# PRBonn/kinematic-icp

Hardware: AMD Instinct MI355X
Metric: scans/sec (ICP registration only), 128k-pt scan vs 1M-pt map (higher is better)
Workload: dtype f64; 1 GPU; cfg2: 131072-pt 64-beam scan vs 986360-pt / 74758-voxel map, voxel 1.00 m, tau 0.6708 m, default ICP iterations (mean 1.00 per scan); one step = one kicp_register_device_batch call = 3200 independent scans against the fixed map, up to 8 in flight at a time (every scan's result bit-identical to registering it alone); 64 distinct scans cycled; scans_in_flight=8, distinct_scans=64, points_per_gpu=131072, parallelism=single GPU

## Files before the change

kinematic_icp_amd/csrc/kicp_kernels.hpp:

```cpp
#pragma once
#include <cfloat>
#include <climits>

#include "kicp_common.hpp"
#include "kicp_se3.hpp"

namespace kicp {

constexpr int kMaxLog = 32;
constexpr int kNumSums = 7;
constexpr int kNumLimbs = 3 * kNumSums;
constexpr int kReduceWords = 24;
constexpr double kFixScale = 1099511627776.0;
constexpr double kFixLimit = 8796093022208.0;

struct HostRecord {
    unsigned long long seq;
    int32_t done, iter, converged, nan_flag;
    Pose T;
    double beta;
    double log_ncorr[kMaxLog];
    double log_sums[kMaxLog][6];
    double log_dx[kMaxLog][2];
    double sums[kNumSums];
// ... 66 lines not shown
    return sp;
}

struct PassParams {
    const double *src;
    uint32_t n;
    MapView map;
    double tau;
    SearchParams search;
    IcpState *st;
    unsigned long long *partials;
    unsigned int *tickets;
    unsigned long long *group_acc;
    SolveParams sol;
    int32_t dbg;
    int32_t *corr_index;
    double *corr_d2, *corr_nn;
};
#ifdef KICP_DBG_BUILD
constexpr bool kDbgBuild = true;
#else
constexpr bool kDbgBuild = false;
#endif
__device__ __forceinline__ bool dbg_is(const PassParams &p, int v) { return kDbgBuild && p.dbg == v; }
__device__ __forceinline__ bool dbg_not(const PassParams &p, int v) { return !kDbgBuild || p.dbg != v; }


struct I128 {
    unsigned long long lo;
    long long hi;
// ... 363 lines not shown
}

__device__ __forceinline__ int wave_sum_to_lane63(int v) {
    v += __builtin_amdgcn_update_dpp(0, v, 0x111, 0xF, 0xF, true);
    v += __builtin_amdgcn_update_dpp(0, v, 0x112, 0xF, 0xF, true);
    v += __builtin_amdgcn_update_dpp(0, v, 0x114, 0xF, 0xF, true);
    v += __builtin_amdgcn_update_dpp(0, v, 0x118, 0xF, 0xF, true);
    v += __builtin_amdgcn_update_dpp(0, v, 0x142, 0xA, 0xF, true);
    v += __builtin_amdgcn_update_dpp(0, v, 0x143, 0xC, 0xF, true);
    return v;
}

constexpr unsigned long long kGaveUpUnit = 1ull << 16;
constexpr unsigned long long kLostRowUnit = 1ull << 8;
constexpr long long kRowWaitTicks = 200000000ll;
__device__ __forceinline__ void counting_hand_over(const I128 &t, int range_error, int gave_up, const PassParams &p, uint32_t row_tag, uint32_t acc_set,
                                                   uint32_t row_set, int lane, uint32_t nblocks = gridDim.x) {
    const uint32_t b = blockIdx.x, g = b / kGroup, ngroups = (nblocks + kGroup - 1) / kGroup;
    long long l[3] = {0ll, 0ll, 0ll};
    if (lane < kNumSums) i128_to_limbs(t, l);
    const int from = min(lane, kNumLimbs - 1) / 3;
    const long long a0 = __shfl(l[0], from, 64), a1 = __shfl(l[1], from, 64), a2 = __shfl(l[2], from, 64);
    long long word = lane % 3 == 0 ? a0 : (lane % 3 == 1 ? a1 : a2);
    if (lane >= kNumLimbs) word = lane == kNumLimbs ? static_cast<long long>(range_error) + (gave_up ? static_cast<long long>(kGaveUpUnit) : 0ll) : 0ll;
    if (lane < kReduceWords) {
        const uint32_t group_size = min(static_cast<uint32_t>(kGroup), nblocks - g * kGroup);
        unsigned long long *acc = p.group_acc + (static_cast<size_t>(acc_set) * ngroups + g) * kAccStride + lane;
        const unsigned long long mine = static_cast<unsigned long long>(word + kAccBias);
        const unsigned long long old = __hip_atomic_fetch_add(acc, (1ull << kAccCountShift) + mine, __ATOMIC_RELAXED, __HIP_MEMORY_SCOPE_AGENT);
        if ((old >> kAccCountShift) == group_size - 1u) {
            const long long total = static_cast<long long>((old & ((1ull << kAccCountShift) - 1ull)) + mine) - static_cast<long long>(group_size) * kAccBias;
            __hip_atomic_store(acc, 0ull, __ATOMIC_RELAXED, __HIP_MEMORY_SCOPE_AGENT);
            __hip_atomic_store(p.sol.pub_rows + (static_cast<size_t>(row_set) * ngroups + g) * kReduceWords + lane,
                               (static_cast<unsigned long long>(total) << 16) | static_cast<unsigned long long>(row_tag), __ATOMIC_RELAXED, __HIP_MEMORY_SCOPE_SYSTEM);
        }
    }
}

template <int BLOCK, bool ROWS_ONLY = false>
__device__ __forceinline__ void finish_pass(Acc &a, const PassParams &p, int (*s_red)[kWaveLimbs], int *s_flag, uint32_t row_tag, int gave_up = 0,
                                            uint32_t parity = 0u, uint32_t nblocks = gridDim.x) {
    const int lane = threadIdx.x & 63, wave = threadIdx.x >> 6;
    IcpState *st = p.st;
    if (!ROWS_ONLY && dbg_is(p, 8)) {
        if (p.sol.mode == 4 && wave == 0 && blockIdx.x % kGroup == 0 && lane < kReduceWords)
            __hip_atomic_store(p.sol.pub_rows + static_cast<size_t>(blockIdx.x / kGroup) * kReduceWords + lane, static_cast<unsigned long long>(p.sol.tag),
                               __ATOMIC_RELAXED, __HIP_MEMORY_SCOPE_SYSTEM);
        if (blockIdx.x == 0 && wave == 0 && p.sol.mode == 2) {
            if (lane < kReduceWords) __hip_atomic_store(p.sol.pub_words + lane, 0ll, __ATOMIC_RELAXED, __HIP_MEMORY_SCOPE_SYSTEM);
            asm volatile("s_waitcnt vmcnt(0)" ::: "memory");
            if (lane == 0) __hip_atomic_store(p.sol.pub_seq, p.sol.pub_value, __ATOMIC_RELAXED, __HIP_MEMORY_SCOPE_SYSTEM);
        }
        return;
    }
    int range_error = a.range_error;
    int limb[kWaveLimbs];
    if (dbg_is(p, 10) || dbg_is(p, 12)) {
#pragma unroll
        for (int k = 0; k < kWaveLimbs; ++k) limb[k] = wave_sum_to_lane63(a.limb[k]);
    } else {
        const unsigned long long holders = __ballot(a.limb[6 * kTermLimbs + 1] != 0);
        const int n_holders = __popcll(holders);
        const int some = holders ? static_cast<int>(__ffsll(static_cast<long long>(holders))) - 1 : 0;
#pragma unroll
        for (int k = 0; k < kTermLimbs; ++k) limb[k] = n_holders * __builtin_amdgcn_readlane(a.limb[k], some);
        limb[6 * kTermLimbs] = 0, limb[6 * kTermLimbs + 1] = n_holders << 19, limb[6 * kTermLimbs + 2] = 0, limb[6 * kTermLimbs + 3] = 0;
        int w10[10], x5[5];
        const bool p0 = (lane & 1) != 0, p1 = (lane & 2) != 0;
#pragma unroll
        for (int j = 0; j < 10; ++j) {
            const int lo = a.limb[kTermLimbs + 2 * j], hi = a.limb[kTermLimbs + 2 * j + 1];
            w10[j] = (p0 ? hi : lo) + __builtin_amdgcn_update_dpp(0, p0 ? lo : hi, 0xB1, 0xF, 0xF, true);
        }
#pragma unroll
        for (int j = 0; j < 5; ++j) {
            const int lo = w10[2 * j], hi = w10[2 * j + 1];
            x5[j] = (p1 ? hi : lo) + __builtin_amdgcn_update_dpp(0, p1 ? lo : hi, 0x4E, 0xF, 0xF, true);
        }
#pragma unroll
        for (int j = 0; j < 5; ++j) x5[j] += __builtin_amdgcn_update_dpp(0, x5[j], 0x114, 0xF, 0xF, true);
// ... 13 lines not shown
            for (int k = 0; k < kTermLimbs; ++k) s_red[wave][k] = limb[k], s_red[wave][6 * kTermLimbs + k] = limb[6 * kTermLimbs + k];
            if (range_error) atomicOr(s_flag, 2);
        }
    }
    if (dbg_is(p, 10) || dbg_is(p, 12)) {
        range_error = __any(range_error) ? 1 : 0;
        if (lane == 63) {
#pragma unroll
            for (int k = 0; k < kWaveLimbs; ++k) s_red[wave][k] = limb[k];
            if (range_error) atomicOr(s_flag, 2);
        }
    }
    __syncthreads();
    if (wave != 0) return;
    range_error = (*s_flag & 2) ? 1 : 0;
    I128 t{0ull, 0ll};
    if (lane < kNumSums) {
        for (int w = 0; w < BLOCK / 64; ++w)
            i128_add_limb_sums(t, s_red[w][kTermLimbs * lane], s_red[w][kTermLimbs * lane + 1], s_red[w][kTermLimbs * lane + 2], s_red[w][kTermLimbs * lane + 3]);
    }
    const uint32_t b = blockIdx.x, g = b / kGroup, ngroups = (nblocks + kGroup - 1) / kGroup;
    const bool counting = ROWS_ONLY || (p.sol.mode == 4 && dbg_not(p, 14));
    if (!ROWS_ONLY && counting) parity = row_tag & 1u;
    if (counting) {
        counting_hand_over(t, range_error, gave_up, p, row_tag, parity, ROWS_ONLY ? parity : 0u, lane, nblocks);
        return;
    }
    unsigned long long *const rows0 = p.partials + (ROWS_ONLY ? static_cast<size_t>(parity) * nblocks * kReduceWords : 0u);
    unsigned int *const tickets0 = p.tickets + (ROWS_ONLY ? static_cast<size_t>(parity) * ngroups * kTicketStride : 0u);
    unsigned long long *row = rows0 + static_cast<size_t>(b) * kReduceWords;
    if (ROWS_ONLY || p.sol.mode == 4 || p.sol.mode == 6) {
        const unsigned long long tag = row_tag;
        if (lane < kNumSums) {
            long long l[3];
            i128_to_limbs(t, l);
#pragma unroll
            for (int j = 0; j < 3; ++j) st_sc1(row + 3 * lane + j, (static_cast<unsigned long long>(l[j]) << 16) | tag);
        } else if (lane < kNumSums + 3) {
            st_sc1(row + kNumLimbs + (lane - kNumSums),
                   ((lane == kNumSums ? static_cast<unsigned long long>(range_error) + (gave_up ? kGaveUpUnit : 0ull) : 0ull) << 16) | tag);
        }
// ... 551 lines not shown
        Best3 o;
        o.b1 = __shfl_xor(L.t.b1, off, 64), o.b2 = __shfl_xor(L.t.b2, off, 64), o.b3 = __shfl_xor(L.t.b3, off, 64);
        o.i1 = __shfl_xor(L.t.i1, off, 64), o.i2 = __shfl_xor(L.t.i2, off, 64), o.o1 = __shfl_xor(L.t.o1, off, 64), o.o2 = __shfl_xor(L.t.o2, off, 64);
        best3_merge(L.t, o);
    }
    if (PARK) {
        kept.q.x = park[0 * BLOCK + tid], kept.q.y = park[1 * BLOCK + tid], kept.q.z = park[2 * BLOCK + tid];
        kept.sx = park[3 * BLOCK + tid], kept.sy = park[4 * BLOCK + tid], kept.voxel = false;
    }
    if (sub == 0) {
        resolve_and_accumulate<EXPORT, ACC, JOBS>(acc, p, host_pose, src, T, L.i, L.t, (LAT || PARK) ? &kept : nullptr);
    }
    if constexpr (ACC::kKind == AccKind::Pass)
        if (dbg_is(p, 10) && (tid & 63u) == 0u) acc.limb[6 * kTermLimbs + 1] = static_cast<int>(rounds & 3u) << 19, acc.limb[6 * kTermLimbs + 2] = static_cast<int>(rounds >> 2);
}
template <int BLOCK, int G, int OCC, bool SPLIT, bool LAT = false, bool EXPORT = false>
__global__ __launch_bounds__(BLOCK, OCC) void k_pass_gather32(const PassParams p) {
    static_assert(!SPLIT || G == 2, "bucket sharing is written for pairs of lanes");
    static_assert(!LAT || G == 1, "the latency-oriented build serves one lane per query");
    KICP_PASS_SHARED(BLOCK)
    constexpr bool kLends = G == 1 && !SPLIT && !LAT;
    __shared__ int s_lend[kLends ? BLOCK / 64 : 1][kLendWords];
    __shared__ double s_park[kLends ? BLOCK * kParkWords : 1];
    const Pose T = load_pose(p);
    const bool host_pose = p.sol.pass == 0 || p.sol.mode >= 2;
    Acc acc{};
    gather32_pass<BLOCK, G, SPLIT, LAT, kLends, EXPORT>(p, T, host_pose, threadIdx.x, acc, p.src, p.n, blockIdx.x, kLends ? &s_lend[kLends ? threadIdx.x / 64 : 0][0] : nullptr,
                                                s_park);
    if (BLOCK > 64) __syncthreads();
    finish_pass<BLOCK>(acc, p, s_red, &s_flag, p.sol.tag);
}
template <int BLOCK, int G, int OCC>
__global__ __launch_bounds__(BLOCK, OCC) void k_pass_gather32_jobs(const JobsParams) {
    static_assert(G == 1, "the job list serves the one-lane-per-query build");
    const uint32_t job = blockIdx.y;
    const uint32_t nblocks = ((JobsKernarg)__builtin_amdgcn_kernarg_segment_ptr())->nblocks[job];
    if (blockIdx.x >= nblocks) return;
    const PassParams &p = job_args(job);
    KICP_PASS_SHARED(BLOCK)
    __shared__ int s_lend[BLOCK / 64][kLendWords];
    __shared__ double s_park[BLOCK * kParkWords];
    const Pose T = p.sol.pose0;
    Acc acc{};
    gather32_pass<BLOCK, G, false, false, true, false, Acc, true>(p, T, true, threadIdx.x, acc, p.src, p.n, blockIdx.x, &s_lend[threadIdx.x / 64][0], s_park);
    __syncthreads();
    finish_pass<BLOCK>(acc, p, s_red, &s_flag, p.sol.tag, 0, 0u, nblocks);
}

static __global__ __launch_bounds__(64) void k_publish_words(IcpState *st, HostRecord *rec, unsigned long long call_id, int pass) {
    const int lane = threadIdx.x;
    if (lane < kReduceWords) __hip_atomic_store(&rec->words[lane], st->reduce[lane], __ATOMIC_RELAXED, __HIP_MEMORY_SCOPE_SYSTEM);
    asm volatile("s_waitcnt vmcnt(0)" ::: "memory");
    if (lane == 0) __hip_atomic_store(&rec->seq, (call_id << 16) | static_cast<unsigned long long>(pass + 1), __ATOMIC_RELAXED, __HIP_MEMORY_SCOPE_SYSTEM);
}

static __global__ __launch_bounds__(64) void k_publish_sums(IcpState *st, HostRecord *rec, unsigned long long call_id) {
    if (threadIdx.x != 0) return;
    for (int i = 0; i < kNumSums; ++i)
        __hip_atomic_store(reinterpret_cast<unsigned long long *>(&rec->sums[i]),
                           static_cast<unsigned long long>(__double_as_longlong(limbs_to_double(st->reduce + 3 * i))), __ATOMIC_RELAXED,
                           __HIP_MEMORY_SCOPE_SYSTEM);
// ... 34 lines not shown
```

kinematic_icp_amd/csrc/kicp_reg_api.hip:

```cpp
#include "kicp_reg_internal.hpp"

using namespace kicp;
using namespace kicp::host;

namespace kicp {
namespace host {
int ensure_frame(kicp_reg *r, size_t n) {
    if (n <= r->d_frame.capacity() / 3) return KICP_OK;
    if (int rc = aql_quiesce(r)) return rc;
    return r->d_frame.reserve((n + n / 4 + 1024) * 3);
}
}
}
namespace {
constexpr size_t kBarFramePoints = 8192;
template <typename T>
__global__ __launch_bounds__(256) void k_fetch_frame(const T *__restrict__ staged, double *__restrict__ dst, uint32_t count) {
    constexpr uint32_t kPer = 16 / sizeof(T);
    const uint32_t i = (blockIdx.x * 256u + threadIdx.x) * kPer;
    if (i + kPer <= count) {
        typedef unsigned int u32x4 __attribute__((ext_vector_type(4)));
        const u32x4 w = __builtin_nontemporal_load(reinterpret_cast<const u32x4 *>(staged + i));
        T v[kPer];
        __builtin_memcpy(v, &w, 16);
// ... 110 lines not shown
    if (k == "timing") {
        reg->timing = static_cast<int>(value);
    }
    else if (k == "wait") reg->wait_mode = static_cast<int>(value);
    else if (k == "debug_p2p_one_row") reg->p2p_rows = value != 0.0 ? 2 : 1;
    else if (k == "debug_tag") reg->tag = static_cast<uint32_t>(value) & 0xFFFFu;
    else if (k == "lanes_per_query") reg->lanes_per_query = (value >= 4) ? 4 : (value >= 2 ? 2 : (value >= 1 ? 1 : 0));
    else if (k == "resident_generic") reg->resident_generic = value != 0.0;
    else if (k == "batch_resident") reg->batch_resident = value != 0.0;
    else if (k == "batch_queues") reg->batch_queues = std::min<int>(std::max(static_cast<int>(value), 0), kMaxBatchInFlight), reg->batch_queues_set = true;
    else if (k == "batch_group") reg->batch_group = std::min<int>(std::max(static_cast<int>(value), 1), kMaxJobs);
    else if (k == "batch_rotate") reg->batch_rotate = value != 0.0;
    else if (k == "batch_threads") reg->batch_threads = std::min<int>(std::max(static_cast<int>(value), 0), kMaxBatchQueues + 1);
    else if (k == "batch_depth") reg->batch_depth = std::min<int>(std::max(static_cast<int>(value), 1), kPipeSlots);
    else if (k == "latency_kernel") reg->latency_kernel = value == 2.0 ? 2 : (value == 1.0 ? 1 : 0);
    else if (k == "aql") reg->use_aql = value != 0.0 ? 1 : 0;
    else if (k == "bar_frame") reg->use_bar_frame = value != 0.0 ? 1 : 0;
    else if (k == "fetch_upload") reg->fetch_frames = value != 0.0 ? 1 : 0;
    else if (k == "small") reg->use_small = value != 0.0 ? 1 : 0;
    else if (k == "small_resident") reg->small_resident = value == 2.0 ? 2 : (value != 0.0 ? 1 : 0);
    else if (k == "small_wave") reg->small_wave = value != 0.0 ? 1 : 0;
    else if (k == "small_trace") {
        if (value != 0.0 && !reg->d_trace.get()) {
            if (int rc = reg->d_trace.reserve(1024 * 4)) return rc;
            HIP_TRY(hipMemset(reg->d_trace.get(), 0, 1024 * 4 * sizeof(long long)));
        }
        reg->trace_pass = value >= 1.0 ? static_cast<uint32_t>(value) : 1u;
        reg->trace_host_us = reg->trace_dev_us = reg->trace_first_us = 0.0, reg->trace_n = reg->trace_first_n = 0;
    }
    else if (k == "small_cmd") {
// ... 22 lines not shown
    if (k == "lanes_per_query") return reg->lanes_per_query;
    if (k == "resident_generic") return reg->resident_generic;
    if (k == "resident_passes") return reg->last_resident_passes;
    if (k == "batch_resident") return reg->batch_resident;
    if (k == "batch_threads") return reg->batch_threads;
    if (k == "batch_threads_active") return reg->last_batch_threads;
    if (k == "batch_depth") return reg->batch_depth;
    if (k == "batch_rotate") return reg->batch_rotate;
    if (k == "batch_queues") return reg->batch_queues;
    if (k == "batch_group") return reg->batch_group;
    if (k == "batch_group_launches") return static_cast<double>(reg->batch_group_launches);
    if (k == "batch_group_aql_launches") return static_cast<double>(reg->batch_group_aql_launches);
    if (k == "batch_queue_passes") return static_cast<double>(reg->batch_queue_passes);
    if (k == "batch_resident_passes") return static_cast<double>(reg->batch_resident_passes);
    if (k == "latency_kernel") return reg->latency_kernel;
    if (k == "timing") return reg->timing;
    if (k == "aql") return reg->use_aql;
    if (k == "aql_kernarg") return !reg->aql.ready ? -1.0 : (std::strcmp(reg->aql.kernarg_place(), "host memory") == 0 ? 0.0 : (std::strcmp(reg->aql.kernarg_place(), "device memory") == 0 ? 1.0 : 2.0));
    if (k == "bar_frame") return reg->bar_frame ? 1.0 : (reg->use_bar_frame ? 0.5 : 0.0);
    if (k == "comm_ranks") {
        int count = 0;
        if (reg->comm && g_comm.CommCount && g_comm.CommCount(reg->comm, &count) == ncclSuccess) return count;
        return reg->comm ? reg->nranks : 0;
    }
    if (k == "fetch_upload") return reg->fetch_frames;
    if (k == "small") return reg->use_small;
    if (k == "small_resident") return reg->small_resident;
    if (k == "small_wave") return reg->small_wave;
    if (k == "trace_host_us") return reg->trace_n ? reg->trace_host_us / static_cast<double>(reg->trace_n) : 0.0;
    if (k == "trace_device_us") return reg->trace_n ? reg->trace_dev_us / static_cast<double>(reg->trace_n) : 0.0;
// ... 164 lines not shown
        if (n > 0x7FFFFFF0ull / 3) return fail(KICP_ERR_CAPACITY, "frame too large");
        if (int rc = ensure_frame(reg, n)) return rc;
        if (int rc = aql_quiesce(reg)) return rc;
        reg->stream_dirty = true;
        if (int rc = fetch_upload<float>(reg, frame_xyz_f32, n)) return rc;
    }
    return run_registration(reg, map, reg->d_frame.get(), n, last_pose_qt, rel_odom_qt, max_correspondence_distance, out_pose_qt, stats);
}
int kicp_reg_clone(const kicp_reg *reg, kicp_reg **out) {
    if (!reg || !out) return fail(KICP_ERR_ARG, "null argument");
    kicp_reg *c = nullptr;
    if (int rc = kicp_reg_create(&reg->cfg, reg->device, &c)) return rc;
    c->use_bar_frame = reg->use_bar_frame, c->fetch_frames = reg->fetch_frames;
    c->wait_mode = reg->wait_mode, c->timing = reg->timing;
    c->query_every = reg->query_every, c->lanes_per_query = reg->lanes_per_query, c->latency_kernel = reg->latency_kernel;
    c->p2p_rows = reg->p2p_rows, c->use_aql = reg->use_aql;
    c->small_cmd = reg->cmd_bar ? 1 : reg->small_cmd, c->use_small = reg->use_small, c->small_block = reg->small_block, c->small_wave = reg->small_wave;
    c->wave_block = reg->wave_block, c->small_resident = reg->small_resident, c->small_timeout_us = reg->small_timeout_us, c->small_group_rows = reg->small_group_rows;
    c->resident_generic = reg->resident_generic, c->batch_resident = reg->batch_resident, c->batch_depth = reg->batch_depth, c->batch_rotate = reg->batch_rotate, c->batch_queues = reg->batch_queues, c->batch_queues_set = reg->batch_queues_set, c->batch_group = reg->batch_group, c->batch_threads = reg->batch_threads ;
    c->score_chunk = reg->score_chunk;
    c->search_max_nodes = reg->search_max_nodes;
    *out = c;
    return KICP_OK;
}
int kicp_pass_correspondences(kicp_reg *reg, kicp_map *map, const double *frame_xyz, size_t n, const double pose_qt[7], double max_correspondence_distance,
                              int32_t *out_index, double *out_d2, double *out_nn_xyz) {
    KICP_TRACE_CALL();
    if (!reg || !map || (!frame_xyz && n) || !pose_qt || (n && (!out_index || !out_d2 || !out_nn_xyz))) return fail(KICP_ERR_ARG, "null argument");
    if (n == 0) return KICP_OK;
    if (n > 0x7FFFFFF0ull / 3) return fail(KICP_ERR_CAPACITY, "frame too large");
// ... 97 lines not shown
```

kinematic_icp_amd/csrc/kicp_reg_batch.hip:

```cpp
#include "kicp_reg_internal.hpp"

using namespace kicp;
using namespace kicp::host;

namespace kicp {
namespace host {
int shm_lane_exchange(kicp_reg *o, int lane, const long long *mine, long long *sum, long long *per_rank) {
    const unsigned long long step = o->shm_lane_step[lane]++;
    kicp_reg::ShmSlot *slots = o->shm + 2 * static_cast<size_t>(o->nranks) * (1 + lane) + (step & 1) * o->nranks;
    for (int i = 0; i < kReduceWords; ++i) slots[o->rank].words[i] = mine[i];
    __atomic_store_n(&slots[o->rank].seq, step + 1, __ATOMIC_RELEASE);
    const Deadline deadline;
    unsigned polls = 0;
    for (int k = 0; k < o->nranks; ++k)
        while (__atomic_load_n(&slots[k].seq, __ATOMIC_ACQUIRE) != step + 1)
            if (++polls % 4096u == 0u && deadline.passed()) return fail(KICP_ERR_COMM, "timed out waiting for a peer rank's hand-off (KICP_WAIT_TIMEOUT_S)");
    for (int i = 0; i < kReduceWords; ++i) sum[i] = 0;
    for (int k = 0; k < o->nranks; ++k)
        for (int i = 0; i < kReduceWords; ++i) {
            sum[i] += slots[k].words[i];
            if (per_rank) per_rank[static_cast<size_t>(k) * kReduceWords + i] = slots[k].words[i];
        }
    return KICP_OK;
}
// ... 243 lines not shown
    threads = static_cast<int>(std::min<size_t>({static_cast<size_t>(threads), count / kMinScansPerThread, fit}));
    if (threads < (wave ? 2 : 3)) return 1;
    if (int rc = set_device(r->device)) return rc;
    if (int rc = map_sync(map, r->device, r->stream)) return rc;
    HIP_TRY(hipStreamSynchronize(r->stream));
    while (static_cast<int>(r->batch_lanes.size()) < threads - 1) {
        kicp_reg *c = nullptr;
        if (int rc = kicp_reg_clone(r, &c)) return rc;
        r->batch_lanes.push_back(c);
    }
    std::vector<kicp_reg *> handles{r};
    std::vector<unsigned long long> passes_before, relaunches_before;
    for (int t = 1; t < threads; ++t) {
        kicp_reg *h = r->batch_lanes[t - 1];
        h->cfg = r->cfg, h->query_every = r->query_every, h->dbg = 0, h->latency_kernel = r->latency_kernel, h->batch_queues = 0, h->batch_threads = 0;
        h->use_small = r->use_small, h->small_wave = r->small_wave, h->wave_block = r->wave_block, h->small_block = r->small_block, h->small_resident = r->small_resident;
        h->small_group_rows = r->small_group_rows, h->small_timeout_us = r->small_timeout_us, h->batch_depth = r->batch_depth, h->batch_rotate = r->batch_rotate;
        h->batch_resident = 1, h->resident_generic = 1, h->small_cmd = r->cmd_bar ? 1 : r->small_cmd;
        handles.push_back(h);
    }
    for (kicp_reg *h : handles) passes_before.push_back(h->batch_resident_passes), relaunches_before.push_back(h->small_relaunches);
    std::vector<int> rcs(static_cast<size_t>(threads), KICP_OK), worsts(static_cast<size_t>(threads), KICP_OK);
    std::vector<std::string> messages(static_cast<size_t>(threads));
    const std::function<void(size_t)> lane = [&](size_t t) {
        kicp_reg *h = handles[t];
        const size_t lo = count * t / static_cast<size_t>(threads), hi = count * (t + 1) / static_cast<size_t>(threads);
        size_t done = 0;
        int rc = run_batch_resident(h, map, hi - lo, d_frames + lo, n + lo, last_poses_qt + 7 * lo, rel_odoms_qt + 7 * lo, tau, out_poses_qt + 7 * lo,
                                    out_iterations ? out_iterations + lo : nullptr, &done, &worsts[t]);
        kicp_stats st;
// ... 25 lines not shown
```

kinematic_icp_amd/csrc/kicp_reg_internal.hpp:

```cpp
#pragma once
#include <dlfcn.h>
#include <fcntl.h>
#include <sched.h>
#include <rccl/rccl.h>
#include <sys/mman.h>
#include <sys/stat.h>
#include <unistd.h>

#include <atomic>
#include <condition_variable>
#include <functional>
#include <mutex>
#include <thread>

#include "kicp_aql.hpp"
#include "kicp_internal.hpp"
#include "kicp_kernels.hpp"
#include "kicp_small.hpp"

using namespace kicp;
using namespace kicp::host;

namespace kicp {
namespace host {
// ... 55 lines not shown
    uint32_t tag = 0;
    DevBuf<double> d_frame;
    HostStage stage;
    double *bar_frame = nullptr;
    int use_bar_frame = 1;
    int fetch_frames = 1;
    bool bar_frame_tried = false;
    int wait_mode = 0;
    int timing = 0;
    int dbg = 0;
    int32_t *corr_index = nullptr;
    double *corr_d2 = nullptr, *corr_nn = nullptr;
    int query_every = 512;
    int lanes_per_query = 0;
    int latency_kernel = 1;
    ncclComm_t lane_comms[8] = {};
    bool lane_comms_failed = false;
    ncclComm_t comm = nullptr;
    int nranks = 1, rank = 0;
    kicp_allreduce_fn allreduce_fn = nullptr;
    void *allreduce_user = nullptr;
    struct ShmSlot {
        unsigned long long seq;
        long long words[kReduceWords];
        unsigned long long pad[7];
    };
    void *shm_base = nullptr;
    ShmSlot *shm = nullptr;
    ShmSlot *d_shm = nullptr;
    size_t shm_bytes = 0;
// ... 118 lines not shown
            nan_flag = range_error ? 2 : 1;
            const int max_it = r->cfg.max_num_iterations;
            for (int j = iter; stats && j < max_it && j < KICP_MAX_LOG_PASSES; ++j) {
                stats->n_corr[j] = 0.0;
                for (int q = 0; q < 6; ++q) stats->sums[j][q] = 0.0;
                stats->dx[j][0] = stats->dx[j][1] = std::nan("");
            }
            iter = max_it;
            return true;
        }
        return iter >= r->cfg.max_num_iterations;
    }
};
double wait_timeout_s();
int lanes_for(const kicp_reg *r, size_t n);
uint32_t pass_grid(const kicp_reg *r, size_t n);
bool aql_up(kicp_reg *r);
const AqlKernel *aql_lookup(kicp_reg *r, int key, const char *demangled_prefix);
const AqlKernel *aql_kernel_for(kicp_reg *r, int b, int g, int occ, bool split, bool lat);
const AqlKernel *aql_resident_kernel_for(kicp_reg *r, bool lat);
const AqlKernel *aql_small_kernel_for(kicp_reg *r, int block, int g, bool wave);
int aql_quiesce(kicp_reg *r);
int launch_pass(kicp_reg *r, const PassParams &p, bool allow_aql = false);
const AqlKernel *aql_jobs_kernel_for(kicp_reg *r);
int launch_jobs(kicp_reg *r, const JobsParams &jp, uint32_t jobs, uint32_t grid_x);
int ensure_partials(kicp_reg *r, size_t blocks);
int ensure_frame(kicp_reg *r, size_t n);
int ensure_rows(kicp_reg *r, size_t groups);
int next_tag(kicp_reg *r, uint32_t *tag);
int enqueue_allreduce(kicp_reg *r);
int wait_record(kicp_reg *r, unsigned long long call_id, unsigned min_iter, bool need_done, unsigned long long *seq_out);
// ... 71 lines not shown
```

kinematic_icp_amd/csrc/kicp_reg_launch.hip:

```cpp
#include "kicp_reg_internal.hpp"

using namespace kicp;
using namespace kicp::host;

namespace kicp {
namespace host {
double host_limbs_to_double(const long long l[3]) {
    unsigned __int128 t = static_cast<unsigned __int128>(static_cast<__int128>(l[0]));
    t += static_cast<unsigned __int128>(static_cast<__int128>(l[1])) << 40;
    t += static_cast<unsigned __int128>(static_cast<__int128>(l[2])) << 80;
    const bool neg = static_cast<__int128>(t) < 0;
    if (neg) t = ~t + 1;
    const double mag = static_cast<double>(static_cast<unsigned long long>(t >> 64)) * 18446744073709551616.0 +
                       static_cast<double>(static_cast<unsigned long long>(t));
    return (neg ? -mag : mag) / kFixScale;
}


double wait_timeout_s() {
    static const double t = [] {
        const char *e = std::getenv("KICP_WAIT_TIMEOUT_S");
        const double v = e ? std::atof(e) : 0.0;
        return v > 0.0 ? v : 20.0;
    }();
    return t;
}


int lanes_for(const kicp_reg *r, size_t n) {
    if (r->lanes_per_query > 0) return r->lanes_per_query;
    return n <= 4096 ? 4 : (n <= 32768 ? 2 : 1);
}
uint32_t pass_grid(const kicp_reg *r, size_t n) {
    const size_t threads = n * static_cast<size_t>(lanes_for(r, n));
    return static_cast<uint32_t>(std::max<size_t>(1, (threads + kPassBlock - 1) / kPassBlock));
}
bool aql_up(kicp_reg *r) {
    if (!r->aql_tried) {
        r->aql_tried = true;
        if (r->aql.init(r->device) != 0 && env_flag("KICP_TRACE")) std::fprintf(stderr, "[kicp] AQL dispatch unavailable: %s\n", r->aql.why.c_str());
        else if (env_flag("KICP_TRACE")) std::fprintf(stderr, "[kicp] AQL dispatch ready, kernel arguments in %s%s%s\n", r->aql.kernarg_place(), r->aql.why.empty() ? "" : "; ", r->aql.why.c_str());
    }
    if (r->aql.ready && r->aql.queue_error) {
        if (env_flag("KICP_TRACE")) std::fprintf(stderr, "[kicp] AQL queue error %d: falling back to the HIP stream\n", r->aql.queue_error);
        r->aql.disable();
    }
    return r->aql.ready;
}
const AqlKernel *aql_lookup(kicp_reg *r, int key, const char *demangled_prefix) {
    if (!aql_up(r)) return nullptr;
// ... 13 lines not shown
const AqlKernel *aql_small_kernel_for(kicp_reg *r, int block, int g, bool wave) {
    char name[128];
    if (wave) std::snprintf(name, sizeof name, "void kicp::k_pass_wave<%d, false>(", block);
    else std::snprintf(name, sizeof name, "void kicp::k_pass_small<%d, %d, false>(", block, g);
    return aql_lookup(r, -(block * 10 + (wave ? 9 : g)), name);
}
int aql_quiesce(kicp_reg *r) {
    if (!r->aql.busy()) return KICP_OK;
    if (r->aql.drain(wait_timeout_s())) return KICP_OK;
    if (r->aql.queue_error) {
        r->aql.disable();
        return KICP_OK;
    }
    return fail(KICP_ERR_HIP, "the AQL queue did not drain (KICP_WAIT_TIMEOUT_S)");
}
int launch_pass(kicp_reg *r, const PassParams &p, bool allow_aql) {
    const uint32_t grid = pass_grid(r, p.n);
    const int g = lanes_for(r, p.n);
    const bool lat = g == 1 && (r->latency_kernel == 2 || (r->latency_kernel == 1 && p.n <= kLatencyMaxPoints));
    const int occ = lat ? 2 : 4;
    const bool split = g == 2;
    if (p.corr_index) {
        if (int rc = aql_quiesce(r)) return rc;
        r->last_via_aql = false;
        if (lat) hipLaunchKernelGGL((k_pass_gather32<kPassBlock, 1, 2, false, true, true>), dim3(grid), dim3(kPassBlock), 0, r->stream, p);
        else if (g == 1) hipLaunchKernelGGL((k_pass_gather32<kPassBlock, 1, 4, false, false, true>), dim3(grid), dim3(kPassBlock), 0, r->stream, p);
        else if (g == 2) hipLaunchKernelGGL((k_pass_gather32<kPassBlock, 2, 4, true, false, true>), dim3(grid), dim3(kPassBlock), 0, r->stream, p);
        else hipLaunchKernelGGL((k_pass_gather32<kPassBlock, 4, 4, false, false, true>), dim3(grid), dim3(kPassBlock), 0, r->stream, p);
        return KICP_OK;
    }
    if (allow_aql && r->use_aql && !r->stream_dirty) {
        if (const AqlKernel *k = aql_kernel_for(r, kPassBlock, g, occ, split, lat)) {
            if (r->aql.dispatch(*k, grid, static_cast<uint32_t>(kPassBlock), &p, sizeof p, HSA_FENCE_SCOPE_AGENT, HSA_FENCE_SCOPE_AGENT)) {
                r->last_via_aql = true;
// ... 347 lines not shown
```

kinematic_icp_amd/csrc/kicp_reg_queues.hip:

```cpp
#include "kicp_reg_internal.hpp"
#include "kicp_batch_groups.hpp"

using namespace kicp;
using namespace kicp::host;

namespace kicp {
namespace host {
static_assert(kMaxBatchQueues == kicp_reg::kShmLanes, "a lane of a sharded batch call owns one area of the shared segment");
struct BatchFlight {
    kicp_reg *h = nullptr;
    HostLoop loop;
    PassParams pp{};
    SmallParams sp{};
    SmallPlan pl;
    bool small = false;
    bool own_rows = false;
    size_t k = 0, rows = 0, row_next = 0;
    uint32_t tag = 0;
    bool active = false;
    unsigned polls = 0;
    long long words[kReduceWords] = {};
    __int128 total[kNumSums] = {};
    unsigned long long flags = 0;
    Deadline since;
// ... 153 lines not shown
    const SearchParams search = search_params(tau, map->mirror.view.voxel_size);
    for (size_t s = 0; s < L.jobs.size(); ++s) {
        GroupJob &j = L.jobs[s];
        PassParams &pp = L.jp.job[s];
        pp = PassParams{};
        pp.src = d_frames[j.k], pp.n = static_cast<uint32_t>(n[j.k]), pp.map = map->mirror.view, pp.tau = tau, pp.st = h->d_state.get();
        pp.search = search, pp.dbg = h->dbg;
        pp.partials = nullptr, pp.tickets = nullptr;
        pp.group_acc = h->d_group_acc.get() + s * 2 * slot_groups * kAccStride;
        SolveParams &sol = pp.sol;
        set_pose(sol, j.loop.T);
        sol.pass = j.loop.iter, sol.mode = 4, sol.max_iterations = h->cfg.max_num_iterations;
        sol.convergence_criterion = h->cfg.convergence_criterion;
        sol.call_id = ++h->call_id, sol.rec = h->rec.dev(), sol.pub_rows = h->rows.dev() + s * slot_groups * kReduceWords;
        sol.tag = j.tag = tag0 + static_cast<uint32_t>(s);
        const uint32_t grid = pass_grid(h, n[j.k]);
        L.jp.nblocks[s] = grid, grid_x = std::max(grid_x, grid);
        j.rows = (grid + kGroup - 1) / kGroup, j.row_next = 0, j.collected = false, j.goes_on = false;
        for (auto &w : j.words) w = 0;
    }
    L.pending = L.jobs.size(), L.polls = 0, L.since = Deadline();
    ++r->batch_group_launches;
    if (int rc = launch_jobs(h, L.jp, static_cast<uint32_t>(L.jobs.size()), grid_x)) return rc;
    if (h->last_via_aql) ++r->batch_group_aql_launches;
    return KICP_OK;
}
static int group_job_rows(GroupLane &L, size_t s, size_t slot_groups) {
    GroupJob &j = L.jobs[s];
    const unsigned long long *base = L.solo.h->rows.get() + s * slot_groups * kReduceWords;
    for (; j.row_next < j.rows; ++j.row_next) {
        const unsigned long long *row = base + j.row_next * kReduceWords;
// ... 9 lines not shown
        j.words[kNumLimbs] |= row_flags(static_cast<long long>(w[kNumLimbs]) >> 16);
    }
    __atomic_thread_fence(__ATOMIC_ACQUIRE);
    return 1;
}
static int run_batch_groups(kicp_reg *r, kicp_map *map, size_t count, const double *const *d_frames, const size_t *n, const double *last_poses_qt,
                            const double *rel_odoms_qt, double tau, double *out_poses_qt, int *out_iterations, size_t *done, int *worst, int lanes, int group) {
    std::vector<GroupLane> L(static_cast<size_t>(lanes));
    std::vector<unsigned char> solo(count, 0);
    size_t slot_groups = 1;
    for (int j = 0; j < lanes; ++j) L[j].solo.h = r->batch_lanes[j];
    kicp_reg *h0 = L[0].solo.h;
    for (size_t k = 0; k < count; ++k) {
        const SmallPlan pl = h0->use_small ? small_plan(h0, n[k]) : SmallPlan();
        solo[k] = (pl.grid != 0 && !pl.generic) || lanes_for(h0, n[k]) != 1;
        if (!solo[k]) slot_groups = std::max<size_t>(slot_groups, (pass_grid(h0, n[k]) + kGroup - 1) / kGroup);
    }
    BatchGroups sched(count, group, solo);
    auto leave = [&](int rc) {
        for (int j = 0; j < lanes; ++j) {
            kicp_reg *h = L[j].solo.h;
            (void)aql_quiesce(h);
            (void)hipStreamSynchronize(h->stream);
            if (rc < 0 && L[j].active) h->acc_dirty = true;
        }
        *done = sched.done();
        return rc;
    };
    auto finish_scan = [&](const HostLoop &loop, size_t k) {
        pose_to(loop.T, out_poses_qt + 7 * k);
        if (out_iterations) out_iterations[k] = loop.iter;
// ... 139 lines not shown
    if (!any_large) return 1;
    if (int rc = set_device(r->device)) return rc;
    const uint64_t epoch_before = map->mirror.synced_epoch;
    if (int rc = map_sync(map, r->device, r->stream)) return rc;
    if (map->mirror.synced_epoch != epoch_before) HIP_TRY(hipStreamSynchronize(r->stream));
    while (static_cast<int>(r->batch_lanes.size()) < lanes) {
        kicp_reg *c = nullptr;
        if (int rc = kicp_reg_clone(r, &c)) return rc;
        r->batch_lanes.push_back(c);
    }
    BatchFlight flights[kMaxBatchQueues];
    for (int j = 0; j < lanes; ++j) {
        kicp_reg *h = r->batch_lanes[j];
        h->cfg = r->cfg, h->lanes_per_query = r->lanes_per_query;
        h->query_every = r->query_every, h->dbg = r->dbg, h->latency_kernel = 0, h->small_resident = 0, h->batch_queues = 0;
        h->small_group_rows = r->small_group_rows;
        h->use_small = sharded ? 0 : r->use_small, h->small_block = r->small_block, h->small_wave = r->small_wave, h->wave_block = r->wave_block;
        flights[j].h = h;
        flights[j].next = static_cast<size_t>(j);
        flights[j].via_comm = over_rccl;
        if (over_rccl) {
            if (!r->lane_comms[j]) {
                const ncclResult_t rc = g_comm.CommSplit(r->comm, 0, r->rank, &r->lane_comms[j], nullptr);
                if (rc != ncclSuccess || !r->lane_comms[j]) {
                    r->lane_comms[j] = nullptr, r->lane_comms_failed = true;
                    for (int i = 0; i < j; ++i) flights[i].h->comm = nullptr;
                    return 1;
                }
            }
            h->comm = r->lane_comms[j], h->nranks = r->nranks, h->rank = r->rank;
// ... 89 lines not shown
```

kinematic_icp_amd/csrc/kicp_small.hpp:

```cpp
#pragma once
#include "kicp_kernels.hpp"

namespace kicp {

constexpr int kSmallMaxLanes = 16384;
constexpr int kSmallMaxGroups = 64;
constexpr int kSmallRowWords = 16;
constexpr uint32_t kSmallMaxPasses = 48;
constexpr int kCmdWords = 8;
enum : uint32_t { kCmdContinue = 1u, kCmdStop = 2u, kCmdNewScan = 3u };
constexpr unsigned long long kCmdMaxScans = 1ull << 24;
constexpr uint32_t kPipeSlots = 4;
struct ScanRef {
    const double *src;
    unsigned long long n;
};
constexpr unsigned long long kSmallGaveUp = 2ull;

KICP_HD unsigned long long cmd_fold(const unsigned long long w[7]) {
    unsigned long long x = 0x9E3779B97F4A7C15ull;
    for (int i = 0; i < 7; ++i) {
        x = (x ^ w[i]) * 0xD6E8FEB86659FD93ull;
        x ^= x >> 32;
    }
// ... 79 lines not shown
template <int BLOCK>
__device__ __forceinline__ void small_publish(const Acc &a, const SmallParams &sp, uint32_t tid, uint32_t pass, int (*s_red)[kWaveLimbs], int *s_flag, int gave_up = 0) {
    const uint32_t tag = sp.tag0 + pass;
    const int lane = tid & 63, wave = tid >> 6;
    int limb[kWaveLimbs];
#pragma unroll
    for (int k = 0; k < kWaveLimbs; ++k) limb[k] = wave_sum_to_lane63(a.limb[k]);
    const int range_error = __any(a.range_error) ? 1 : 0;
    if (lane == 63) {
#pragma unroll
        for (int k = 0; k < kWaveLimbs; ++k) s_red[wave][k] = limb[k];
        if (range_error) atomicOr(s_flag, 2);
    }
    __syncthreads();
    if (wave != 0) return;
    I128 t{0ull, 0ll};
    if (lane < kNumSums)
        for (int w = 0; w < BLOCK / 64; ++w)
            i128_add_limb_sums(t, s_red[w][kTermLimbs * lane], s_red[w][kTermLimbs * lane + 1], s_red[w][kTermLimbs * lane + 2], s_red[w][kTermLimbs * lane + 3]);
    if (sp.group_rows) {
        counting_hand_over(t, (*s_flag & 2) ? 1 : 0, gave_up, sp.p, tag, pass % kPipeSlots, pass % kPipeSlots, lane);
        return;
    }
    const unsigned long long m48 = (1ull << 48) - 1;
    const unsigned long long h0 = t.lo & m48, h1 = ((t.lo >> 48) | (static_cast<unsigned long long>(t.hi) << 16)) & m48;
    const unsigned long long v0 = __shfl(h0, lane >> 1, 64), v1 = __shfl(h1, lane >> 1, 64);
    unsigned long long word = (lane & 1) ? v1 : v0;
    if (lane == 2 * kNumSums) word = (*s_flag & 2) ? 1ull : 0ull;
    if (lane > 2 * kNumSums) word = 0ull;
    if (lane < kSmallRowWords)
        __hip_atomic_store(sp.rows + (static_cast<size_t>(pass % kPipeSlots) * gridDim.x + blockIdx.x) * kSmallRowWords + lane, (word << 16) | tag, __ATOMIC_RELAXED,
                           __HIP_MEMORY_SCOPE_SYSTEM);
}

template <int BLOCK, int G, bool EXPORT = false>
__global__ __launch_bounds__(BLOCK) void k_pass_small(const SmallParams ) {
    __shared__ int s_red[BLOCK / 64][kWaveLimbs];
    __shared__ int s_flag;
// ... 376 lines not shown
```

Measured before the change: 189,100 scans/s.

## Let each pass workgroup process several tiles and shrink grid accordingly

```diff
diff --git a/kinematic_icp_amd/csrc/kicp_kernels.hpp b/kinematic_icp_amd/csrc/kicp_kernels.hpp
--- a/kinematic_icp_amd/csrc/kicp_kernels.hpp
+++ b/kinematic_icp_amd/csrc/kicp_kernels.hpp
@@ -3,6 +3,7 @@
 #include <climits>
 
 #include "kicp_common.hpp"
+#include "kicp_pass_tiles.hpp"
 #include "kicp_se3.hpp"
 
 namespace kicp {
@@ -104,6 +105,7 @@
     unsigned long long *group_acc;
     SolveParams sol;
     int32_t dbg;
+    uint32_t tiles;
     int32_t *corr_index;
     double *corr_d2, *corr_nn;
 };
@@ -497,11 +499,9 @@
 constexpr unsigned long long kGaveUpUnit = 1ull << 16;
 constexpr unsigned long long kLostRowUnit = 1ull << 8;
 constexpr long long kRowWaitTicks = 200000000ll;
-__device__ __forceinline__ void counting_hand_over(const I128 &t, int range_error, int gave_up, const PassParams &p, uint32_t row_tag, uint32_t acc_set,
+__device__ __forceinline__ void counting_hand_over(const long long (&l)[3], int range_error, int gave_up, const PassParams &p, uint32_t row_tag, uint32_t acc_set,
                                                    uint32_t row_set, int lane, uint32_t nblocks = gridDim.x) {
     const uint32_t b = blockIdx.x, g = b / kGroup, ngroups = (nblocks + kGroup - 1) / kGroup;
-    long long l[3] = {0ll, 0ll, 0ll};
-    if (lane < kNumSums) i128_to_limbs(t, l);
     const int from = min(lane, kNumLimbs - 1) / 3;
     const long long a0 = __shfl(l[0], from, 64), a1 = __shfl(l[1], from, 64), a2 = __shfl(l[2], from, 64);
     long long word = lane % 3 == 0 ? a0 : (lane % 3 == 1 ? a1 : a2);
@@ -519,10 +519,28 @@
         }
     }
 }
-
-template <int BLOCK, bool ROWS_ONLY = false>
+__device__ __forceinline__ void counting_hand_over(const I128 &t, int range_error, int gave_up, const PassParams &p, uint32_t row_tag, uint32_t acc_set,
+                                                   uint32_t row_set, int lane, uint32_t nblocks = gridDim.x) {
+    long long l[3] = {0ll, 0ll, 0ll};
+    if (lane < kNumSums) i128_to_limbs(t, l);
+    counting_hand_over(l, range_error, gave_up, p, row_tag, acc_set, row_set, lane, nblocks);
+}
+template <int WAVES>
+__device__ __forceinline__ void workgroup_row_words(const int (*s_red)[kWaveLimbs], int lane, long long (&l)[3]) {
+    l[0] = l[1] = l[2] = 0ll;
+    if (lane < kNumSums) {
+        long long s[kTermLimbs] = {0ll, 0ll, 0ll, 0ll};
+#pragma unroll
+        for (int w = 0; w < WAVES; ++w)
+#pragma unroll
+            for (int k = 0; k < kTermLimbs; ++k) s[k] += s_red[w][kTermLimbs * lane + k];
+        limb_sums_to_words(s[0], s[1], s[2], s[3], l);
+    }
+}
+
+template <int BLOCK, bool ROWS_ONLY = false, bool TILED = false>
 __device__ __forceinline__ void finish_pass(Acc &a, const PassParams &p, int (*s_red)[kWaveLimbs], int *s_flag, uint32_t row_tag, int gave_up = 0,
-                                            uint32_t parity = 0u, uint32_t nblocks = gridDim.x) {
+                                            uint32_t parity = 0u, uint32_t nblocks = gridDim.x, int holders = 0, const int *jtj = nullptr) {
     const int lane = threadIdx.x & 63, wave = threadIdx.x >> 6;
     IcpState *st = p.st;
     if (!ROWS_ONLY && dbg_is(p, 8)) {
@@ -542,11 +560,18 @@
 #pragma unroll
         for (int k = 0; k < kWaveLimbs; ++k) limb[k] = wave_sum_to_lane63(a.limb[k]);
     } else {
-        const unsigned long long holders = __ballot(a.limb[6 * kTermLimbs + 1] != 0);
-        const int n_holders = __popcll(holders);
-        const int some = holders ? static_cast<int>(__ffsll(static_cast<long long>(holders))) - 1 : 0;
-#pragma unroll
-        for (int k = 0; k < kTermLimbs; ++k) limb[k] = n_holders * __builtin_amdgcn_readlane(a.limb[k], some);
+        int n_holders;
+        if constexpr (TILED) {
+            n_holders = holders;
+#pragma unroll
+            for (int k = 0; k < kTermLimbs; ++k) limb[k] = n_holders * jtj[k];
+        } else {
+            const unsigned long long held = __ballot(a.limb[6 * kTermLimbs + 1] != 0);
+            n_holders = __popcll(held);
+            const int some = held ? static_cast<int>(__ffsll(static_cast<long long>(held))) - 1 : 0;
+#pragma unroll
+            for (int k = 0; k < kTermLimbs; ++k) limb[k] = n_holders * __builtin_amdgcn_readlane(a.limb[k], some);
+        }
         limb[6 * kTermLimbs] = 0, limb[6 * kTermLimbs + 1] = n_holders << 19, limb[6 * kTermLimbs + 2] = 0, limb[6 * kTermLimbs + 3] = 0;
         int w10[10], x5[5];
         const bool p0 = (lane & 1) != 0, p1 = (lane & 2) != 0;
@@ -590,17 +615,19 @@
     __syncthreads();
     if (wave != 0) return;
     range_error = (*s_flag & 2) ? 1 : 0;
+    const uint32_t b = blockIdx.x, g = b / kGroup, ngroups = (nblocks + kGroup - 1) / kGroup;
+    const bool counting = ROWS_ONLY || (p.sol.mode == 4 && dbg_not(p, 14));
+    if (!ROWS_ONLY && counting) parity = row_tag & 1u;
+    if (counting) {
+        long long l[3];
+        workgroup_row_words<BLOCK / 64>(s_red, lane, l);
+        counting_hand_over(l, range_error, gave_up, p, row_tag, parity, ROWS_ONLY ? parity : 0u, lane, nblocks);
+        return;
+    }
     I128 t{0ull, 0ll};
     if (lane < kNumSums) {
         for (int w = 0; w < BLOCK / 64; ++w)
             i128_add_limb_sums(t, s_red[w][kTermLimbs * lane], s_red[w][kTermLimbs * lane + 1], s_red[w][kTermLimbs * lane + 2], s_red[w][kTermLimbs * lane + 3]);
-    }
-    const uint32_t b = blockIdx.x, g = b / kGroup, ngroups = (nblocks + kGroup - 1) / kGroup;
-    const bool counting = ROWS_ONLY || (p.sol.mode == 4 && dbg_not(p, 14));
-    if (!ROWS_ONLY && counting) parity = row_tag & 1u;
-    if (counting) {
-        counting_hand_over(t, range_error, gave_up, p, row_tag, parity, ROWS_ONLY ? parity : 0u, lane, nblocks);
-        return;
     }
     unsigned long long *const rows0 = p.partials + (ROWS_ONLY ? static_cast<size_t>(parity) * nblocks * kReduceWords : 0u);
     unsigned int *const tickets0 = p.tickets + (ROWS_ONLY ? static_cast<size_t>(parity) * ngroups * kTicketStride : 0u);
@@ -1182,6 +1209,57 @@
     if constexpr (ACC::kKind == AccKind::Pass)
         if (dbg_is(p, 10) && (tid & 63u) == 0u) acc.limb[6 * kTermLimbs + 1] = static_cast<int>(rounds & 3u) << 19, acc.limb[6 * kTermLimbs + 2] = static_cast<int>(rounds >> 2);
 }
+constexpr int kTileLimbs = kWaveLimbs - 2 * kTermLimbs;
+template <int BLOCK, bool EXPORT, bool JOBS>
+__device__ __forceinline__ int pass_tiles_loop(Acc &acc, int (*lend)[kLendWords], double *park, int (*tile)[BLOCK]) {
+    const uint32_t tid = threadIdx.x;
+    int holders = 0, range_error = 0;
+    uint32_t block = blockIdx.x;
+    for (;;) {
+        asm volatile("; kept in vector registers through the tile" : "+v"(holders), "+v"(range_error));
+        const PassParams &pt = JOBS ? job_args_at_point_of_use(blockIdx.y) : args_at_point_of_use();
+        const Pose T = JOBS ? pt.sol.pose0 : load_pose(pt);
+        const bool host_pose = JOBS || pt.sol.pass == 0 || pt.sol.mode >= 2;
+        uint32_t lane_id = tid;
+        asm volatile("; a tile starts here" : "+v"(lane_id));
+        Acc one{};
+        gather32_pass<BLOCK, 1, false, false, true, EXPORT, Acc, JOBS>(pt, T, host_pose, lane_id, one, pt.src, pt.n, block, &lend[lane_id / 64u][0], park);
+        holders += __popcll(__ballot(one.limb[6 * kTermLimbs + 1] != 0));
+        range_error |= one.range_error;
+        const PassParams &pe = JOBS ? job_args_at_point_of_use(blockIdx.y) : args_at_point_of_use();
+        const uint32_t tiles = min(pe.tiles, static_cast<uint32_t>(kMaxPassTiles));
+        if (tiles <= 1u) {
+            acc = one;
+            break;
+        }
+        if (block == blockIdx.x) {
+#pragma unroll
+            for (int k = 0; k < kTileLimbs; ++k) tile[k][tid] = one.limb[kTermLimbs + k];
+        } else {
+#pragma unroll
+            for (int k = 0; k < kTileLimbs; ++k) (void)__hip_atomic_fetch_add(&tile[k][tid], one.limb[kTermLimbs + k], __ATOMIC_RELAXED, __HIP_MEMORY_SCOPE_WAVEFRONT);
+        }
+        const uint32_t nwg = JOBS ? ((JobsKernarg)__builtin_amdgcn_kernarg_segment_ptr())->nblocks[blockIdx.y] : gridDim.x;
+        const uint32_t end = min((pe.n + BLOCK - 1) / BLOCK, blockIdx.x + tiles * nwg);
+        block += nwg;
+        if (block >= end) {
+#pragma unroll
+            for (int k = 0; k < kTileLimbs; ++k) acc.limb[kTermLimbs + k] = tile[k][tid];
+            break;
+        }
+    }
+    acc.range_error = range_error;
+    return __builtin_amdgcn_readfirstlane(holders);
+}
+template <bool JOBS>
+__device__ __forceinline__ void pass_jtj00(int (&jtj)[kTermLimbs]) {
+    const PassParams &p = JOBS ? job_args_at_point_of_use(blockIdx.y) : args_at_point_of_use();
+    PassBasis B;
+    if (JOBS || p.sol.pass == 0 || p.sol.mode >= 2) B = p.sol.basis;
+    else B = basis_of(load_pose(p));
+#pragma unroll
+    for (int k = 0; k < kTermLimbs; ++k) jtj[k] = B.jtj00[k];
+}
 template <int BLOCK, int G, int OCC, bool SPLIT, bool LAT = false, bool EXPORT = false>
 __global__ __launch_bounds__(BLOCK, OCC) void k_pass_gather32(const PassParams p) {
     static_assert(!SPLIT || G == 2, "bucket sharing is written for pairs of lanes");
@@ -1190,13 +1268,22 @@
     constexpr bool kLends = G == 1 && !SPLIT && !LAT;
     __shared__ int s_lend[kLends ? BLOCK / 64 : 1][kLendWords];
     __shared__ double s_park[kLends ? BLOCK * kParkWords : 1];
-    const Pose T = load_pose(p);
-    const bool host_pose = p.sol.pass == 0 || p.sol.mode >= 2;
     Acc acc{};
-    gather32_pass<BLOCK, G, SPLIT, LAT, kLends, EXPORT>(p, T, host_pose, threadIdx.x, acc, p.src, p.n, blockIdx.x, kLends ? &s_lend[kLends ? threadIdx.x / 64 : 0][0] : nullptr,
-                                                s_park);
-    if (BLOCK > 64) __syncthreads();
-    finish_pass<BLOCK>(acc, p, s_red, &s_flag, p.sol.tag);
+    if constexpr (kLends) {
+        __shared__ int s_tile[kTileLimbs][BLOCK];
+        const int holders = pass_tiles_loop<BLOCK, EXPORT, false>(acc, s_lend, s_park, s_tile);
+        int jtj[kTermLimbs];
+        pass_jtj00<false>(jtj);
+        __syncthreads();
+        const PassParams &pf = args_at_point_of_use();
+        finish_pass<BLOCK, false, true>(acc, pf, s_red, &s_flag, pf.sol.tag, 0, 0u, gridDim.x, holders, jtj);
+    } else {
+        const Pose T = load_pose(p);
+        const bool host_pose = p.sol.pass == 0 || p.sol.mode >= 2;
+        gather32_pass<BLOCK, G, SPLIT, LAT, kLends, EXPORT>(p, T, host_pose, threadIdx.x, acc, p.src, p.n, blockIdx.x, nullptr, s_park);
+        if (BLOCK > 64) __syncthreads();
+        finish_pass<BLOCK>(acc, p, s_red, &s_flag, p.sol.tag);
+    }
 }
 template <int BLOCK, int G, int OCC>
 __global__ __launch_bounds__(BLOCK, OCC) void k_pass_gather32_jobs(const JobsParams) {
@@ -1208,11 +1295,13 @@
     KICP_PASS_SHARED(BLOCK)
     __shared__ int s_lend[BLOCK / 64][kLendWords];
     __shared__ double s_park[BLOCK * kParkWords];
-    const Pose T = p.sol.pose0;
+    __shared__ int s_tile[kTileLimbs][BLOCK];
     Acc acc{};
-    gather32_pass<BLOCK, G, false, false, true, false, Acc, true>(p, T, true, threadIdx.x, acc, p.src, p.n, blockIdx.x, &s_lend[threadIdx.x / 64][0], s_park);
+    const int holders = pass_tiles_loop<BLOCK, false, true>(acc, s_lend, s_park, s_tile);
+    int jtj[kTermLimbs];
+    pass_jtj00<true>(jtj);
     __syncthreads();
-    finish_pass<BLOCK>(acc, p, s_red, &s_flag, p.sol.tag, 0, 0u, nblocks);
+    finish_pass<BLOCK, false, true>(acc, p, s_red, &s_flag, p.sol.tag, 0, 0u, nblocks, holders, jtj);
 }
 
 static __global__ __launch_bounds__(64) void k_publish_words(IcpState *st, HostRecord *rec, unsigned long long call_id, int pass) {
diff --git a/kinematic_icp_amd/csrc/kicp_pass_tiles.hpp b/kinematic_icp_amd/csrc/kicp_pass_tiles.hpp
--- /dev/null
+++ b/kinematic_icp_amd/csrc/kicp_pass_tiles.hpp
@@ -0,0 +1,31 @@
+#pragma once
+#include <algorithm>
+#include <cstddef>
+#include <cstdint>
+
+#if defined(__HIPCC__)
+#define KICP_TILES_HD __host__ __device__ __forceinline__
+#else
+#define KICP_TILES_HD inline
+#endif
+
+namespace kicp {
+constexpr int kMaxPassTiles = 4;
+KICP_TILES_HD void limb_sums_to_words(long long s0, long long s1, long long s2, long long s3, long long w[3]) {
+    const long long low = s0 + s1 * 2097152ll;
+    const long long s3h = (s3 + 65536ll) >> 17, s3l = s3 - s3h * 131072ll;
+    w[0] = low & ((1ll << 40) - 1ll);
+    w[1] = (low >> 40) + s2 * 4ll + s3l * 8388608ll;
+    w[2] = s3h;
+}
+
+namespace host {
+inline uint32_t auto_pass_tiles(size_t blocks, int in_flight, int cus) {
+    const size_t slots = 4u * static_cast<size_t>(std::max(1, cus)), scans = static_cast<size_t>(std::max(1, in_flight));
+    for (uint32_t t = static_cast<uint32_t>(kMaxPassTiles); t > 1u; t /= 2u)
+        if (2u * ((blocks + t - 1u) / t) * scans >= 3u * slots) return t;
+    return 1u;
+}
+inline int clamp_pass_tiles(double value) { return value >= 4.0 ? 4 : (value >= 2.0 ? 2 : (value >= 1.0 ? 1 : 0)); }
+}
+}
diff --git a/kinematic_icp_amd/csrc/kicp_reg_api.hip b/kinematic_icp_amd/csrc/kicp_reg_api.hip
--- a/kinematic_icp_amd/csrc/kicp_reg_api.hip
+++ b/kinematic_icp_amd/csrc/kicp_reg_api.hip
@@ -148,6 +148,7 @@
     else if (k == "batch_threads") reg->batch_threads = std::min<int>(std::max(static_cast<int>(value), 0), kMaxBatchQueues + 1);
     else if (k == "batch_depth") reg->batch_depth = std::min<int>(std::max(static_cast<int>(value), 1), kPipeSlots);
     else if (k == "latency_kernel") reg->latency_kernel = value == 2.0 ? 2 : (value == 1.0 ? 1 : 0);
+    else if (k == "pass_tiles") reg->pass_tiles = clamp_pass_tiles(value);
     else if (k == "aql") reg->use_aql = value != 0.0 ? 1 : 0;
     else if (k == "bar_frame") reg->use_bar_frame = value != 0.0 ? 1 : 0;
     else if (k == "fetch_upload") reg->fetch_frames = value != 0.0 ? 1 : 0;
@@ -200,6 +201,7 @@
     if (k == "batch_queue_passes") return static_cast<double>(reg->batch_queue_passes);
     if (k == "batch_resident_passes") return static_cast<double>(reg->batch_resident_passes);
     if (k == "latency_kernel") return reg->latency_kernel;
+    if (k == "pass_tiles") return reg->pass_tiles;
     if (k == "timing") return reg->timing;
     if (k == "aql") return reg->use_aql;
     if (k == "aql_kernarg") return !reg->aql.ready ? -1.0 : (std::strcmp(reg->aql.kernarg_place(), "host memory") == 0 ? 0.0 : (std::strcmp(reg->aql.kernarg_place(), "device memory") == 0 ? 1.0 : 2.0));
@@ -394,6 +396,7 @@
     c->use_bar_frame = reg->use_bar_frame, c->fetch_frames = reg->fetch_frames;
     c->wait_mode = reg->wait_mode, c->timing = reg->timing;
     c->query_every = reg->query_every, c->lanes_per_query = reg->lanes_per_query, c->latency_kernel = reg->latency_kernel;
+    c->pass_tiles = reg->pass_tiles;
     c->p2p_rows = reg->p2p_rows, c->use_aql = reg->use_aql;
     c->small_cmd = reg->cmd_bar ? 1 : reg->small_cmd, c->use_small = reg->use_small, c->small_block = reg->small_block, c->small_wave = reg->small_wave;
     c->wave_block = reg->wave_block, c->small_resident = reg->small_resident, c->small_timeout_us = reg->small_timeout_us, c->small_group_rows = reg->small_group_rows;
diff --git a/kinematic_icp_amd/csrc/kicp_reg_batch.hip b/kinematic_icp_amd/csrc/kicp_reg_batch.hip
--- a/kinematic_icp_amd/csrc/kicp_reg_batch.hip
+++ b/kinematic_icp_amd/csrc/kicp_reg_batch.hip
@@ -281,6 +281,7 @@
     for (int t = 1; t < threads; ++t) {
         kicp_reg *h = r->batch_lanes[t - 1];
         h->cfg = r->cfg, h->query_every = r->query_every, h->dbg = 0, h->latency_kernel = r->latency_kernel, h->batch_queues = 0, h->batch_threads = 0;
+        h->pass_tiles = r->pass_tiles, h->scans_in_flight = 1;
         h->use_small = r->use_small, h->small_wave = r->small_wave, h->wave_block = r->wave_block, h->small_block = r->small_block, h->small_resident = r->small_resident;
         h->small_group_rows = r->small_group_rows, h->small_timeout_us = r->small_timeout_us, h->batch_depth = r->batch_depth, h->batch_rotate = r->batch_rotate;
         h->batch_resident = 1, h->resident_generic = 1, h->small_cmd = r->cmd_bar ? 1 : r->small_cmd;
diff --git a/kinematic_icp_amd/csrc/kicp_reg_internal.hpp b/kinematic_icp_amd/csrc/kicp_reg_internal.hpp
--- a/kinematic_icp_amd/csrc/kicp_reg_internal.hpp
+++ b/kinematic_icp_amd/csrc/kicp_reg_internal.hpp
@@ -93,6 +93,8 @@
     int query_every = 512;
     int lanes_per_query = 0;
     int latency_kernel = 1;
+    int pass_tiles = 0;
+    int scans_in_flight = 1;
     ncclComm_t lane_comms[8] = {};
     bool lane_comms_failed = false;
     ncclComm_t comm = nullptr;
@@ -241,7 +243,8 @@
 };
 double wait_timeout_s();
 int lanes_for(const kicp_reg *r, size_t n);
-uint32_t pass_grid(const kicp_reg *r, size_t n);
+uint32_t pass_tiles(const kicp_reg *r, size_t n, bool jobs = false);
+uint32_t pass_grid(const kicp_reg *r, size_t n, bool jobs = false);
 bool aql_up(kicp_reg *r);
 const AqlKernel *aql_lookup(kicp_reg *r, int key, const char *demangled_prefix);
 const AqlKernel *aql_kernel_for(kicp_reg *r, int b, int g, int occ, bool split, bool lat);
diff --git a/kinematic_icp_amd/csrc/kicp_reg_launch.hip b/kinematic_icp_amd/csrc/kicp_reg_launch.hip
--- a/kinematic_icp_amd/csrc/kicp_reg_launch.hip
+++ b/kinematic_icp_amd/csrc/kicp_reg_launch.hip
@@ -31,9 +31,21 @@
     if (r->lanes_per_query > 0) return r->lanes_per_query;
     return n <= 4096 ? 4 : (n <= 32768 ? 2 : 1);
 }
-uint32_t pass_grid(const kicp_reg *r, size_t n) {
+static bool latency_build_for(const kicp_reg *r, size_t n) {
+    return lanes_for(r, n) == 1 && (r->latency_kernel == 2 || (r->latency_kernel == 1 && n <= kLatencyMaxPoints));
+}
+static size_t pass_blocks(const kicp_reg *r, size_t n) {
     const size_t threads = n * static_cast<size_t>(lanes_for(r, n));
-    return static_cast<uint32_t>(std::max<size_t>(1, (threads + kPassBlock - 1) / kPassBlock));
+    return std::max<size_t>(1, (threads + kPassBlock - 1) / kPassBlock);
+}
+uint32_t pass_tiles(const kicp_reg *r, size_t n, bool jobs) {
+    if (r->dbg != 0 || lanes_for(r, n) != 1 || (!jobs && latency_build_for(r, n))) return 1u;
+    if (r->pass_tiles > 0) return static_cast<uint32_t>(std::min(r->pass_tiles, kMaxPassTiles));
+    return auto_pass_tiles(pass_blocks(r, n), r->scans_in_flight, r->num_cus);
+}
+uint32_t pass_grid(const kicp_reg *r, size_t n, bool jobs) {
+    const size_t tiles = pass_tiles(r, n, jobs);
+    return static_cast<uint32_t>((pass_blocks(r, n) + tiles - 1) / tiles);
 }
 bool aql_up(kicp_reg *r) {
     if (!r->aql_tried) {
@@ -77,10 +89,12 @@
     }
     return fail(KICP_ERR_HIP, "the AQL queue did not drain (KICP_WAIT_TIMEOUT_S)");
 }
-int launch_pass(kicp_reg *r, const PassParams &p, bool allow_aql) {
+int launch_pass(kicp_reg *r, const PassParams &args, bool allow_aql) {
+    PassParams p = args;
+    p.tiles = pass_tiles(r, p.n);
     const uint32_t grid = pass_grid(r, p.n);
     const int g = lanes_for(r, p.n);
-    const bool lat = g == 1 && (r->latency_kernel == 2 || (r->latency_kernel == 1 && p.n <= kLatencyMaxPoints));
+    const bool lat = latency_build_for(r, p.n);
     const int occ = lat ? 2 : 4;
     const bool split = g == 2;
     if (p.corr_index) {
diff --git a/kinematic_icp_amd/csrc/kicp_reg_queues.hip b/kinematic_icp_amd/csrc/kicp_reg_queues.hip
--- a/kinematic_icp_amd/csrc/kicp_reg_queues.hip
+++ b/kinematic_icp_amd/csrc/kicp_reg_queues.hip
@@ -191,7 +191,8 @@
         sol.convergence_criterion = h->cfg.convergence_criterion;
         sol.call_id = ++h->call_id, sol.rec = h->rec.dev(), sol.pub_rows = h->rows.dev() + s * slot_groups * kReduceWords;
         sol.tag = j.tag = tag0 + static_cast<uint32_t>(s);
-        const uint32_t grid = pass_grid(h, n[j.k]);
+        pp.tiles = pass_tiles(h, n[j.k], true);
+        const uint32_t grid = pass_grid(h, n[j.k], true);
         L.jp.nblocks[s] = grid, grid_x = std::max(grid_x, grid);
         j.rows = (grid + kGroup - 1) / kGroup, j.row_next = 0, j.collected = false, j.goes_on = false;
         for (auto &w : j.words) w = 0;
@@ -231,7 +232,7 @@
     for (size_t k = 0; k < count; ++k) {
         const SmallPlan pl = h0->use_small ? small_plan(h0, n[k]) : SmallPlan();
         solo[k] = (pl.grid != 0 && !pl.generic) || lanes_for(h0, n[k]) != 1;
-        if (!solo[k]) slot_groups = std::max<size_t>(slot_groups, (pass_grid(h0, n[k]) + kGroup - 1) / kGroup);
+        if (!solo[k]) slot_groups = std::max<size_t>(slot_groups, (pass_grid(h0, n[k], true) + kGroup - 1) / kGroup);
     }
     BatchGroups sched(count, group, solo);
     auto leave = [&](int rc) {
@@ -401,6 +402,7 @@
         kicp_reg *h = r->batch_lanes[j];
         h->cfg = r->cfg, h->lanes_per_query = r->lanes_per_query;
         h->query_every = r->query_every, h->dbg = r->dbg, h->latency_kernel = 0, h->small_resident = 0, h->batch_queues = 0;
+        h->pass_tiles = r->pass_tiles, h->scans_in_flight = group > 1 ? lanes * group : lanes;
         h->small_group_rows = r->small_group_rows;
         h->use_small = sharded ? 0 : r->use_small, h->small_block = r->small_block, h->small_wave = r->small_wave, h->wave_block = r->wave_block;
         flights[j].h = h;
diff --git a/kinematic_icp_amd/csrc/kicp_small.hpp b/kinematic_icp_amd/csrc/kicp_small.hpp
--- a/kinematic_icp_amd/csrc/kicp_small.hpp
+++ b/kinematic_icp_amd/csrc/kicp_small.hpp
@@ -117,14 +117,16 @@
     }
     __syncthreads();
     if (wave != 0) return;
+    if (sp.group_rows) {
+        long long l[3];
+        workgroup_row_words<BLOCK / 64>(s_red, lane, l);
+        counting_hand_over(l, (*s_flag & 2) ? 1 : 0, gave_up, sp.p, tag, pass % kPipeSlots, pass % kPipeSlots, lane);
+        return;
+    }
     I128 t{0ull, 0ll};
     if (lane < kNumSums)
         for (int w = 0; w < BLOCK / 64; ++w)
             i128_add_limb_sums(t, s_red[w][kTermLimbs * lane], s_red[w][kTermLimbs * lane + 1], s_red[w][kTermLimbs * lane + 2], s_red[w][kTermLimbs * lane + 3]);
-    if (sp.group_rows) {
-        counting_hand_over(t, (*s_flag & 2) ? 1 : 0, gave_up, sp.p, tag, pass % kPipeSlots, pass % kPipeSlots, lane);
-        return;
-    }
     const unsigned long long m48 = (1ull << 48) - 1;
     const unsigned long long h0 = t.lo & m48, h1 = ((t.lo >> 48) | (static_cast<unsigned long long>(t.hi) << 16)) & m48;
     const unsigned long long v0 = __shfl(h0, lane >> 1, 64), v1 = __shfl(h1, lane >> 1, 64);
```

Measured after the change: 203,800 scans/s (median of 6 runs). 1.08x the previous value.
